# guptakhil/show-tell

Measured on AMD Instinct MI355X. Metric: training images/sec (ResNet101+GRU, emb=512, bs=128) at 1/2/4/8 MI355X, higher is better.
Workload: dtype bf16; 1 GPU; BASELINE configs[1]: ResNet-101 (train-mode BN, frozen) + 5-layer GRU decoder, E=H=512, V=10000, fwd+bwd+SGD step, synthetic COCO-shaped batch; batch_per_gpu=128, global_batch=128, image=3x224x224, parallelism=dp1

## Files before the change

include/showtell_hip.h:

```cpp
#ifndef SHOWTELL_HIP_H
#define SHOWTELL_HIP_H

#include <stddef.h>
#include <stdint.h>

#ifdef __cplusplus
extern "C" {
#endif

#define ST_F32 0
#define ST_BF16 1

#define ST_CELL_GRU 0
#define ST_CELL_LSTM 1

const char* st_last_error(void);
int st_version(void);

typedef struct {
  const void* x;
  const void* w;
  void* y;
  const float* bias;
  const float* scale;
// ... 168 lines not shown

int st_cast2d(const void* x, void* y, int from_dtype, int to_dtype, int rows, int cols, int ldx, int ldy, void* stream);

#define ST_MAX_LAYERS 8
typedef struct {
  int cell, dtype, L, in0, H, V, E;
  const void* emb;
  const void* w_ih[ST_MAX_LAYERS]; const void* w_hh[ST_MAX_LAYERS];
  const float* b_ih[ST_MAX_LAYERS]; const float* b_hh[ST_MAX_LAYERS];
  const void* w_lin; const float* b_lin;
} st_rnn_params;

typedef struct {
  float* emb;
  float* w_ih[ST_MAX_LAYERS]; float* w_hh[ST_MAX_LAYERS]; float* b_ih[ST_MAX_LAYERS]; float* b_hh[ST_MAX_LAYERS];
  float* w_lin; float* b_lin;
} st_rnn_grads;

typedef struct {
  int B, T, ntok, Tcap;
  const int* batch_sizes_host;
  const int* rows_b; const int* rows_t; const int* prev_row;
  const long* caption;
} st_packed_seq;

int st_rnn_vocab_ld(int V);
size_t st_rnn_workspace_bytes(const st_rnn_params* p, const st_packed_seq* s);
int st_rnn_forward(const st_rnn_params* p, const st_packed_seq* s, const void* x0_override, const void* feat,
                   void* workspace, size_t workspace_bytes, void* logits, int logits_dtype, int ldl,
                   long* targets, int save_for_backward, void* stream);
int st_rnn_backward(const st_rnn_params* p, const st_rnn_grads* g, const st_packed_seq* s,
                    const void* x0_override, const void* dlogits, int ldd, const float* dy_top,
                    void* workspace, size_t workspace_bytes, float* dfeat, float* dx0_out, void* stream);

int st_rnn_fused_loss_supported(const st_rnn_params* p);
size_t st_rnn_fused_loss_bytes(const st_rnn_params* p, const st_packed_seq* s);
int st_rnn_fused_loss(const st_rnn_params* p, const st_packed_seq* s, const void* workspace, size_t workspace_bytes,
                      const long* targets, float* scratch, size_t scratch_bytes, float* loss_accum, void* stream);
int st_rnn_fused_dlogits(const st_rnn_params* p, const st_packed_seq* s, const void* workspace, size_t workspace_bytes,
                         const long* targets, const float* scratch, const float* grad_scale_dev, void* dlogits, int ldd, void* stream);

int st_cross_entropy(const void* logits, int logits_dtype, const long* target, int rows, int V, int ldl,
                     float* loss_accum, void* dlogits, int dlogits_dtype, int ldd, float grad_scale,
                     const float* grad_scale_dev , void* stream);

size_t st_head_workspace_bytes(int B, int F, int E, int dtype);
int st_linear_bn1d_forward(const void* x, const void* w, const float* bias, const float* gamma, const float* beta,
                           float* running_mean, float* running_var, int B, int F, int E, int dtype,
                           int train, float momentum, float eps,
                           float* z_out, float* save_mean, float* save_rstd, void* y_dtype, float* y_f32, void* stream);
int st_linear_bn1d_backward(const float* dy, const float* z, const void* x, const float* gamma,
                            const float* save_mean, const float* save_rstd, int B, int F, int E, int dtype, int train,
                            float* dw, float* dbias, float* dgamma, float* dbeta, void* workspace, size_t workspace_bytes,
                            void* stream);

int st_sgd_step(float* param, const float* grad, float* momentum_buf, void* bf16_shadow, long n,
                float lr, float momentum, int first_step, float grad_scale, void* stream);
int st_adam_step(float* param, const float* grad, float* exp_avg, float* exp_avg_sq, void* bf16_shadow, long n,
                 float lr, float beta1, float beta2, float eps, int step, float grad_scale, void* stream);

size_t st_rnn_greedy_workspace_bytes(const st_rnn_params* p, int B);
int st_rnn_greedy(const st_rnn_params* p, const void* feat, int B, int steps, void* workspace, size_t workspace_bytes,
                  long* ids_out, float* logits_out, void* stream);
int st_rnn_greedy_last_route(void);

int st_rnn_step(const st_rnn_params* p, const void* x, int n, const void* h_in, const void* c_in,
// ... 47 lines not shown
```

show-tell_amd/_lib.py:

```python
import ctypes as C
import os

_HERE = os.path.dirname(os.path.abspath(__file__))
LIB_PATH = os.path.join(_HERE, "lib", "libshowtell_hip.so")

ST_F32, ST_BF16 = 0, 1
ST_CELL_GRU, ST_CELL_LSTM = 0, 1

c_p, c_i, c_f, c_l = C.c_void_p, C.c_int, C.c_float, C.c_long


class ConvDesc(C.Structure):
    _fields_ = [("x", c_p), ("w", c_p), ("y", c_p), ("bias", c_p), ("scale", c_p), ("shift", c_p),
                ("residual", c_p), ("stats", c_p), ("dtype", c_i), ("out_dtype", c_i),
                ("B", c_i), ("Hin", c_i), ("Win", c_i), ("Cin", c_i), ("Ho", c_i), ("Wo", c_i), ("N", c_i),
                ("KH", c_i), ("KW", c_i), ("stride", c_i), ("pad", c_i),
                ("ldx", c_i), ("ldw", c_i), ("ldy", c_i), ("relu", c_i), ("accumulate", c_i), ("Cin_logical", c_i), ("k_order", c_i), ("stats_replicas", c_i),
                ("in_stats", c_p), ("in_gamma", c_p), ("in_beta", c_p), ("in_count", c_f), ("in_eps", c_f), ("split_k", c_i)]


class Conv3x3ImgDesc(C.Structure):
    _fields_ = [("x", c_p), ("w_frag", c_p), ("y", c_p), ("stats", c_p), ("stats_replicas", c_i), ("scale", c_p), ("shift", c_p),
                ("relu", c_i), ("in_stats", c_p), ("in_gamma", c_p), ("in_beta", c_p), ("in_count", c_f), ("in_eps", c_f),
                ("B", c_i), ("H", c_i), ("W", c_i), ("C", c_i), ("N", c_i), ("in_stats_replicas", c_i)]
# ... 103 lines not shown
    "st_conv1x1_kstream": ([C.POINTER(Conv1x1WregDesc), c_p], c_i),
    "st_pack_conv_weight_frag": ([c_p, c_p, c_i, c_i, c_i, c_i, c_i, c_p], c_i),
    "st_tune": ([c_i, c_i, c_i], c_i),
    "st_prof_enable": ([c_i], c_i),
    "st_debug_stamps": ([c_p], c_i),
    "st_prof_collect": ([C.POINTER(C.c_double), C.POINTER(C.c_double), C.POINTER(c_l)], c_i),
    "st_bn_act": ([C.POINTER(BnActDesc), c_p], c_i),
    "st_bn_update_running": ([c_p, c_p, c_p, c_i, c_f, c_f, c_p], c_i),
    "st_nchw_to_nhwc": ([c_p, c_p, c_i, c_i, c_i, c_i, c_i, c_i, c_p], c_i),
    "st_nchw_to_s2d16": ([c_p, c_p, c_i, c_i, c_i, c_i, c_p], c_i),
    "st_stem_weight_s2d": ([c_p, c_p, c_i, c_i, c_p], c_i),
    "st_stem_weight_frag": ([c_p, c_p, c_p], c_i),
    "st_stem_weight_frag_packed": ([c_p, c_i, c_p, c_p], c_i),
    "st_stem_conv_pool": ([C.POINTER(StemConvPoolDesc), c_p], c_i),
    "st_nhwc_to_ncp_f32": ([c_p, c_p, c_i, c_i, c_i, c_i, c_p], c_i),
    "st_maxpool3x3s2": ([c_p, c_p, c_i, c_i, c_i, c_i, c_i, c_p], c_i),
    "st_maxpool3x3s2_bn": ([c_p, c_p, c_i, c_i, c_i, c_i, c_i, c_p, c_p, c_p, c_p, c_p, c_f, c_f, c_p], c_i),
    "st_global_avgpool": ([c_p, c_p, c_i, c_i, c_i, c_i, c_i, c_p], c_i),
    "st_cast": ([c_p, c_p, c_i, c_i, c_l, c_p], c_i),
    "st_transpose": ([c_p, c_p, c_i, c_i, c_i, c_i, c_i, c_p], c_i),
    "st_transpose_colsum": ([c_p, c_p, c_p, c_i, c_i, c_i, c_i, c_i, c_p], c_i),
    "st_transpose_batch": ([c_p, c_p, c_p, c_i, c_i, c_i, c_i, c_i, c_i, c_p, c_p, c_p], c_i),
    "st_pack_conv_weight": ([c_p, c_p, c_i, c_i, c_i, c_i, c_i, c_i, c_i, c_p], c_i),
    "st_cast2d": ([c_p, c_p, c_i, c_i, c_i, c_i, c_i, c_i, c_p], c_i),
    "st_rnn_vocab_ld": ([c_i], c_i),
    "st_rnn_workspace_bytes": ([C.POINTER(RnnParams), C.POINTER(PackedSeq)], C.c_size_t),
    "st_rnn_forward": ([C.POINTER(RnnParams), C.POINTER(PackedSeq), c_p, c_p, c_p, C.c_size_t, c_p, c_i, c_i, c_p, c_i, c_p], c_i),
    "st_rnn_fused_loss_supported": ([C.POINTER(RnnParams)], c_i),
    "st_rnn_fused_loss_bytes": ([C.POINTER(RnnParams), C.POINTER(PackedSeq)], C.c_size_t),
    "st_rnn_fused_loss": ([C.POINTER(RnnParams), C.POINTER(PackedSeq), c_p, C.c_size_t, c_p, c_p, C.c_size_t, c_p, c_p], c_i),
    "st_rnn_fused_dlogits": ([C.POINTER(RnnParams), C.POINTER(PackedSeq), c_p, C.c_size_t, c_p, c_p, c_p, c_p, c_i, c_p], c_i),
    "st_rnn_backward": ([C.POINTER(RnnParams), C.POINTER(RnnGrads), C.POINTER(PackedSeq), c_p, c_p, c_i, c_p, c_p, C.c_size_t,
                         c_p, c_p, c_p], c_i),
    "st_rnn_greedy_workspace_bytes": ([C.POINTER(RnnParams), c_i], C.c_size_t),
    "st_rnn_greedy": ([C.POINTER(RnnParams), c_p, c_i, c_i, c_p, C.c_size_t, c_p, c_p, c_p], c_i),
    "st_rnn_greedy_last_route": ([], c_i),
    "st_rnn_step": ([C.POINTER(RnnParams), c_p, c_i, c_p, c_p, c_p, c_p, c_p, c_i, c_p], c_i),
    "st_embedding_rows": ([c_p, c_p, c_p, c_i, c_i, c_i, c_i, c_i, c_p], c_i),
    "st_gather_state": ([c_p, c_p, c_p, c_i, c_i, c_i, c_i, c_i, c_p], c_i),
    "st_softmax_topk": ([c_p, c_i, c_i, c_i, c_i, c_p, c_p, c_i, c_p], c_i),
    "st_beam_select": ([c_p, c_p, c_p, c_p, c_p, c_i, c_i, c_i, c_l, c_p, c_p, c_p, c_p, c_p, c_p], c_i),
    "st_attn_workspace_bytes": ([c_p, c_p], C.c_size_t),
    "st_attn_forward": ([c_p, c_p, c_p, c_p, c_p, C.c_size_t, c_p, c_i, c_i, c_p, c_i, c_p], c_i),
    "st_attn_backward": ([c_p, c_p, c_p, c_p, c_p, c_i, c_p, c_p, c_f, c_p, c_p, C.c_size_t, c_p], c_i),
    "st_attn_reg_loss": ([c_p, c_i, c_i, c_i, c_f, c_p, c_p], c_i),
    "st_attn_greedy_workspace_bytes": ([c_p, c_i], C.c_size_t),
    "st_attn_greedy": ([c_p, c_p, c_i, c_i, c_l, c_p, C.c_size_t, c_p, c_p], c_i),
    "st_attn_greedy_alphas": ([c_p, c_p, c_i, c_i, c_l, c_p, C.c_size_t, c_p, c_p, c_p], c_i),
    "st_attn_beam_workspace_bytes": ([c_p, c_i, c_i], C.c_size_t),
    "st_attn_beam_search": ([c_p, c_p, c_i, c_i, c_i, c_l, c_l, c_p, C.c_size_t, c_p, c_p, c_p, c_p, c_p, c_p], c_i),
    "st_cross_entropy": ([c_p, c_i, c_p, c_i, c_i, c_i, c_p, c_p, c_i, c_i, c_f, c_p, c_p], c_i),
    "st_head_workspace_bytes": ([c_i, c_i, c_i, c_i], C.c_size_t),
    "st_linear_bn1d_forward": ([c_p] * 7 + [c_i, c_i, c_i, c_i, c_i, c_f, c_f] + [c_p] * 6, c_i),
    "st_linear_bn1d_backward": ([c_p] * 6 + [c_i, c_i, c_i, c_i, c_i] + [c_p] * 5 + [C.c_size_t, c_p], c_i),
    "st_sgd_step": ([c_p, c_p, c_p, c_p, c_l, c_f, c_f, c_i, c_f, c_p], c_i),
    "st_adam_step": ([c_p, c_p, c_p, c_p, c_p, c_l, c_f, c_f, c_f, c_f, c_i, c_f, c_p], c_i),
    "st_resnet_create": ([c_i, c_i, C.POINTER(c_p)], c_i),
    "st_resnet_destroy": ([c_p], None),
    "st_resnet_num_convs": ([c_p], c_i),
    "st_resnet_feat_dim": ([c_p], c_i),
    "st_resnet_weight_elems": ([c_p], C.c_size_t),
    "st_resnet_bn_channels": ([c_p], C.c_size_t),
    "st_resnet_conv_info": ([c_p, c_i] + [C.POINTER(c_i)] * 6 + [C.POINTER(C.c_size_t)] * 2 + [C.POINTER(c_i), C.POINTER(C.c_size_t), C.POINTER(c_i)], c_i),
    "st_resnet_workspace_bytes": ([c_p, c_i, c_i, c_i], C.c_size_t),
    "st_resnet_set_taps": ([c_p, c_p, C.c_size_t], c_i),
    "st_resnet_forward": ([c_p, c_p, c_i, c_i, c_i, c_p, c_p, c_p, c_p, c_p, c_i, c_f, c_f, c_p, C.c_size_t,
# ... 47 lines not shown
```

show-tell_amd/csrc/rnn.cpp:

```cpp
#include "common.h"
#include "rnn_kernels.h"
#include <string.h>
#include <vector>

namespace {

inline size_t al(size_t v) { return (v + 255) & ~(size_t)255; }
inline int up8(int v) { return (v + 7) & ~7; }

struct Plan {
  int G, GH, Np, Vp, maxw;
  size_t es;
  size_t x0, y, gates, cst, dyl, dx0, dgx, dgh, dhc, dcc, tA, tB, wT, wThh, wTih, gA, gB, total;
};

Plan make_plan(const st_rnn_params* p, const st_packed_seq* s) {
  Plan q;
  q.G = p->cell == ST_CELL_GRU ? 3 : 4;
  q.GH = q.G * p->H;
  q.Np = up8(s->ntok);
  q.Vp = st_rnn_vocab_ld(p->V);
  q.es = st_dtype_size(p->dtype);
  q.maxw = p->in0 > p->H ? p->in0 : p->H;
  const size_t n = s->ntok, L = p->L, H = p->H;
  size_t o = 0;
  auto take = [&](size_t bytes) { size_t r = o; o += al(bytes); return r; };
  q.x0 = take(n * p->in0 * q.es);
  q.y = take(L * n * H * q.es);
  q.gates = take(L * n * 4 * H * q.es);
  q.cst = take(p->cell == ST_CELL_LSTM ? L * n * H * q.es : 0);
  q.dyl = take(L * n * H * sizeof(float));
  q.dx0 = take(n * p->in0 * sizeof(float));
  q.dgx = take(L * n * q.GH * q.es);
  q.dgh = take(p->cell == ST_CELL_GRU ? L * n * q.GH * q.es : 0);
// ... 113 lines not shown
}

extern "C" int st_rnn_fused_loss_supported(const st_rnn_params* p) {
  return p && p->w_lin && p->b_lin && vocab_ce_supported(p->dtype, p->H) ? 1 : 0;
}
extern "C" size_t st_rnn_fused_loss_bytes(const st_rnn_params* p, const st_packed_seq* s) {
  if (!p || !s) return 0;
  return ((size_t)s->ntok * (2 + 2 * (size_t)vocab_ce_tiles(p->V))) * sizeof(float);
}
extern "C" int st_rnn_fused_loss(const st_rnn_params* p, const st_packed_seq* s, const void* workspace, size_t workspace_bytes,
                                 const long* targets, float* scratch, size_t scratch_bytes, float* loss_accum, void* stream) {
  if (check_common(p, s, "st_rnn_fused_loss")) return 1;
  ST_CHECK(workspace && targets && scratch && loss_accum, "st_rnn_fused_loss: null pointer");
  ST_CHECK(st_rnn_fused_loss_supported(p), "st_rnn_fused_loss: needs bf16, H = 512 and the vocabulary projection (use st_rnn_forward's logits + st_cross_entropy)");
  const Plan q = make_plan(p, s);
  ST_CHECK(workspace_bytes >= q.total && scratch_bytes >= st_rnn_fused_loss_bytes(p, s), "st_rnn_fused_loss: workspace / scratch too small");
  const char* ytop = reinterpret_cast<const char*>(workspace) + q.y + (size_t)(p->L - 1) * s->ntok * p->H * q.es;
  const int n = s->ntok;
  return vocab_ce_forward(ytop, p->w_lin, p->b_lin, targets, n, p->V, scratch + 2 * (size_t)n, scratch + n, scratch, loss_accum,
                          reinterpret_cast<hipStream_t>(stream));
}
extern "C" int st_rnn_fused_dlogits(const st_rnn_params* p, const st_packed_seq* s, const void* workspace, size_t workspace_bytes,
                                    const long* targets, const float* scratch, const float* grad_scale_dev, void* dlogits, int ldd, void* stream) {
  if (check_common(p, s, "st_rnn_fused_dlogits")) return 1;
  ST_CHECK(workspace && targets && scratch && dlogits, "st_rnn_fused_dlogits: null pointer");
  ST_CHECK(st_rnn_fused_loss_supported(p), "st_rnn_fused_dlogits: unsupported configuration");
  const Plan q = make_plan(p, s);
  ST_CHECK(workspace_bytes >= q.total, "st_rnn_fused_dlogits: workspace too small");
  const char* ytop = reinterpret_cast<const char*>(workspace) + q.y + (size_t)(p->L - 1) * s->ntok * p->H * q.es;
  return vocab_ce_dlogits(ytop, p->w_lin, p->b_lin, targets, scratch, s->ntok, p->V, dlogits, ldd, 1.0f, grad_scale_dev,
                          reinterpret_cast<hipStream_t>(stream));
}

extern "C" int st_rnn_backward(const st_rnn_params* p, const st_rnn_grads* g, const st_packed_seq* s,
                               const void* x0_override, const void* dlogits, int ldd, const float* dy_top_extra,
                               void* workspace, size_t workspace_bytes, float* dfeat, float* dx0_out, void* stream) {
  if (check_common(p, s, "st_rnn_backward")) return 1;
  ST_CHECK(g && workspace, "st_rnn_backward: null pointer");
  const Plan q = make_plan(p, s);
  ST_CHECK(workspace_bytes >= q.total, "st_rnn_backward: workspace too small (%zu < %zu)", workspace_bytes, q.total);
  hipStream_t st = reinterpret_cast<hipStream_t>(stream);
  char* ws = reinterpret_cast<char*>(workspace);
  const int dt = p->dtype, H = p->H, n = s->ntok, Np = q.Np, GH = q.GH;
  const size_t es = q.es;
  std::vector<int> off(s->T + 1, 0);
  for (int t = 0; t < s->T; ++t) off[t + 1] = off[t] + s->batch_sizes_host[t];
  const int L = p->L, T = s->T;
  auto dyl = [&](int l) { return reinterpret_cast<float*>(ws + q.dyl) + (size_t)l * n * H; };
  float* dy = dyl(L - 1);
  const char* ytop = ws + q.y + (size_t)(p->L - 1) * n * H * es;

  if (dlogits) {
    ST_CHECK(p->w_lin && g->w_lin && g->b_lin, "st_rnn_backward: vocabulary projection gradients requested without buffers");
    ST_CHECK(ldd >= up8(p->V) && ldd % 8 == 0 && ldd <= q.Vp, "st_rnn_backward: dlogits leading dimension %d must be a multiple of 8 in [%d, %d]",
             ldd, up8(p->V), q.Vp);
    if (st_transpose_colsum(dlogits, ws + q.tA, g->b_lin, dt, n, p->V, ldd, Np, stream)) return 1;
    if (st_transpose(ytop, ws + q.tB, dt, n, H, H, Np, stream)) return 1;
    if (gemm_nt(ws + q.tA, Np, ws + q.tB, Np, g->w_lin, H, p->V, H, Np, dt, ST_F32, nullptr, 1, stream)) return 1;
    if (st_transpose(p->w_lin, ws + q.wT, dt, p->V, H, H, ldd, stream)) return 1;
    const int bk = dt == ST_BF16 ? 64 : 32;
    const int split = (ldd % (8 * bk) == 0 && ldd >= 16 * bk) ? 8 : 0;
    if (gemm_nt(dlogits, ldd, ws + q.wT, ldd, dy, H, n, H, ldd, dt, ST_F32, nullptr, 0, stream, split)) return 1;
    if (dy_top_extra) { st_set_error("st_rnn_backward: dlogits and dy_top_extra are exclusive"); return 1; }
  } else {
    ST_CHECK(dy_top_extra, "st_rnn_backward: need dlogits or dy_top");
    if (hipMemcpyAsync(dy, dy_top_extra, (size_t)n * H * sizeof(float), hipMemcpyDeviceToDevice, st) != hipSuccess) {
      st_set_error("st_rnn_backward: copy failed"); return 1;
    }
  }

  const void* x0 = x0_override ? x0_override : ws + q.x0;
  const bool need_dx0 = dfeat || dx0_out || g->emb;
  float* dx0 = dx0_out ? dx0_out : reinterpret_cast<float*>(ws + q.dx0);
  const bool gru = p->cell == ST_CELL_GRU;
  auto dgxl = [&](int l) { return ws + q.dgx + (size_t)l * n * GH * es; };
  auto dghl = [&](int l) { return gru ? ws + q.dgh + (size_t)l * n * GH * es : dgxl(l); };
  auto dhcl = [&](int l) { return reinterpret_cast<float*>(ws + q.dhc) + (size_t)l * s->B * H; };
  auto dccl = [&](int l) { return reinterpret_cast<float*>(ws + q.dcc) + (size_t)l * s->B * H; };
  auto wThh = [&](int l) { return ws + q.wThh + (size_t)l * H * GH * es; };
  auto wTih = [&](int l) { return ws + q.wTih + (size_t)l * q.maxw * GH * es; };
  if (hipMemsetAsync(ws + q.dhc, 0, (size_t)L * s->B * H * sizeof(float), st) != hipSuccess ||
      hipMemsetAsync(ws + q.dcc, 0, (size_t)L * s->B * H * sizeof(float), st) != hipSuccess) { st_set_error("memset failed"); return 1; }
  {
    const void* wx[2][ST_MAX_LAYERS]; void* wy[2][ST_MAX_LAYERS];
    int ni = 0;
    for (int l = 0; l < L; ++l) {
      const int in = l == 0 ? p->in0 : H;
      wx[0][l] = p->w_hh[l]; wy[0][l] = wThh(l);
      if (!(l > 0 || need_dx0)) continue;
      if (in == H) { wx[1][ni] = p->w_ih[l]; wy[1][ni] = wTih(l); ++ni; }
      else if (st_transpose(p->w_ih[l], wTih(l), dt, GH, in, in, GH, stream)) return 1;
    }
    if (st_transpose_batch(wx[0], wy[0], nullptr, L, dt, GH, H, H, GH, nullptr, nullptr, stream)) return 1;
    if (ni && st_transpose_batch(wx[1], wy[1], nullptr, ni, dt, GH, H, H, GH, nullptr, nullptr, stream)) return 1;
  }
  for (int d = T + L - 2; d >= 0; --d) {
    RnnBwdCell gc[ST_MAX_LAYERS];
    RnnGemmArgs mc[2 * ST_MAX_LAYERS];
    int ng = 0, nm = 0;
    for (int l = d < T ? 0 : d - (T - 1); l <= d && l < L; ++l) {
      const int t = d - l;
      const int bt = s->batch_sizes_host[t];
      const int in = l == 0 ? p->in0 : H;
      char* yl = ws + q.y + (size_t)l * n * H * es;
      char* gl = ws + q.gates + (size_t)l * n * 4 * H * es;
      char* cl = ws + q.cst + (size_t)l * n * H * es;
      RnnBwdCell& c = gc[ng++];
      memset(&c, 0, sizeof(c));
      c.dy = dyl(l) + (size_t)off[t] * H; c.dhc = dhcl(l); c.dcc = dccl(l);
      c.cache = gl + (size_t)off[t] * 4 * H * es;
      c.hprev = t > 0 ? yl + (size_t)off[t - 1] * H * es : nullptr;
      c.cnew = cl + (size_t)off[t] * H * es;
      c.cprev = t > 0 ? cl + (size_t)off[t - 1] * H * es : nullptr;
      c.dgx = dgxl(l) + (size_t)off[t] * GH * es; c.dgh = dghl(l) + (size_t)off[t] * GH * es; c.Bt = bt;
      if (t > 0) {
        RnnGemmArgs& a = mc[nm++];
        memset(&a, 0, sizeof(a));
        a.A = dghl(l) + (size_t)off[t] * GH * es; a.W = wThh(l); a.M = bt; a.N = H; a.K = GH; a.lda = GH; a.ldw = GH;
        a.out_f32 = dhcl(l); a.ldo = H; a.accumulate = 1;
      }
      if (l > 0 || need_dx0) {
        RnnGemmArgs& a = mc[nm++];
        memset(&a, 0, sizeof(a));
        a.A = dgxl(l) + (size_t)off[t] * GH * es; a.W = wTih(l); a.M = bt; a.N = in; a.K = GH; a.lda = GH; a.ldw = GH;
        a.out_f32 = (l > 0 ? dyl(l - 1) + (size_t)off[t] * H : dx0 + (size_t)off[t] * in); a.ldo = in;
      }
    }
    if (rnn_bwd_gates_launch_batch(gc, ng, H, p->cell, dt, st)) return 1;
    if (rnn_gemm_launch_batch(mc, nm, dt, 0, 0, st)) return 1;
// ... 50 lines not shown
```

show-tell_amd/csrc/rnn_kernels.h:

```cpp
#pragma once
#include "common.h"

struct RnnGemmArgs {
  const void* A; const void* W; int M, N, K, lda, ldw, gstride;
  const void* A2; const void* W2; int K2, lda2, ldw2;
  float* out_f32; int ldo; int accumulate;
  const float* bias_h; const float* bias_x;
  const void* gx; int ldgx;
  const void* hprev; const void* cprev; int ldhp;
  void* hout; void* cout; int ldho;
  void* hout2; int ldho2;
  void* cache; int ldcache;
  unsigned long long* argmax_keys;
  const unsigned long long* x_keys; int x_V;
  long* ids_out; int ids_stride, ids_t;
};
constexpr int kCellRawOut = 1, kCellSplit = 2;

constexpr int kRnnBatch = 16;
struct RnnGemmBatch { RnnGemmArgs c[kRnnBatch]; };
static_assert(sizeof(RnnGemmBatch) <= 4000, "kernel-argument segment is 4 KiB");
struct RnnBwdCell {
  const float* dy; float* dhc; float* dcc; const void* cache; const void* hprev; const void* cnew; const void* cprev;
  void* dgx; void* dgh; int Bt;
};
struct RnnBwdBatch { RnnBwdCell c[kRnnBatch]; };

#ifdef __HIPCC__
__device__ __forceinline__ float st_sigm(float x) { return 1.0f / (1.0f + expf(-x)); }
__device__ __forceinline__ float st_gru_unit(float xr, float xz, float xn, float hr, float hz, float hn, float hprev, float& r, float& z, float& n) {
  r = st_sigm(xr + hr);
  z = st_sigm(xz + hz);
  n = tanhf(__builtin_fmaf(r, hn, xn));
  return __builtin_fmaf(z, hprev, (1.f - z) * n);
}
__device__ __forceinline__ float st_lstm_unit(float pi, float pf, float pg, float po, float cprev, float& ig, float& fg, float& gg, float& og, float& cn) {
  ig = st_sigm(pi); fg = st_sigm(pf); gg = tanhf(pg); og = st_sigm(po);
  cn = __builtin_fmaf(fg, cprev, ig * gg);
  return og * tanhf(cn);
}
#endif

size_t rnn_greedy_pipe_bytes(const st_rnn_params* p, int B, int steps);
int rnn_greedy_pipe(const st_rnn_params* p, const void* feat, int B, int steps, void* ws, size_t ws_bytes, long* ids_out, hipStream_t st);

int vocab_ce_supported(int dtype, int H);
int vocab_ce_tiles(int V);
int vocab_ce_forward(const void* y, const void* w, const float* bias, const long* target, int n, int V, float* partial, float* tgt,
                     float* lse, float* loss, hipStream_t st);
int vocab_ce_dlogits(const void* y, const void* w, const float* bias, const long* target, const float* lse, int n, int V,
                     void* dlogits, int ldd, float gscale, const float* gscale_dev, hipStream_t st);

int rnn_gemm_launch(const RnnGemmArgs& a, int dtype, int epi, int has_x, hipStream_t st);
int rnn_gemm_launch_batch(const RnnGemmArgs* cells, int ncells, int dtype, int epi, int has_x, hipStream_t st);
int rnn_bwd_gates_launch_batch(const RnnBwdCell* cells, int ncells, int H, int cell_kind, int dtype, hipStream_t st);
int pack_inputs_launch(const void* feat, const void* emb, const long* cap, int Tcap, const int* rows_b, const int* rows_t,
                       void* x0, long* target, int ntok, int E, int V, int mode, int dtype, hipStream_t st);
int embedding_bwd_launch(const float* dx0, const long* cap, int Tcap, const int* rows_b, const int* rows_t,
                         float* dfeat, float* demb, int ntok, int E, int V, int mode, hipStream_t st);
int gather_hprev_launch(const void* y, const int* rows_t, const int* prev_row, void* hp, int ntok, int H, int dtype, hipStream_t st,
                        const void* h0 = nullptr, const int* rows_b = nullptr);
int gru_bwd_gates_launch(const float* dy, float* dhc, const void* cache, const void* hprev, void* dgx, void* dgh,
                         int Bt, int H, int dtype, hipStream_t st);
int lstm_bwd_gates_launch(const float* dy, float* dhc, float* dcc, const void* cache, const void* cnew, const void* cprev,
                          void* dg, int Bt, int H, int dtype, hipStream_t st);
int colsum_launch(const void* x, float* out, int rows, int cols, int ldx, int dtype, hipStream_t st);
```

show-tell_amd/csrc/rnn_kernels.hip:

```cpp
#include "common.h"
#include "rnn_kernels.h"
#include <string.h>

namespace {

template <typename T> struct Mfma;
template <> struct Mfma<bf16_t> {
  static constexpr int EPC = 8;
  static __device__ __forceinline__ void run(const u32x4& a, const u32x4& b, f32x4& c) {
    c = __builtin_amdgcn_mfma_f32_16x16x32_bf16(*reinterpret_cast<const bf16x8*>(&a),
                                                *reinterpret_cast<const bf16x8*>(&b), c, 0, 0, 0);
  }
};
template <> struct Mfma<float> {
  static constexpr int EPC = 4;
  static __device__ __forceinline__ void run(const u32x4& a, const u32x4& b, f32x4& c) {
#pragma unroll
    for (int e = 0; e < 4; ++e)
      c = __builtin_amdgcn_mfma_f32_16x16x4f32(__uint_as_float(a[e]), __uint_as_float(b[e]), c, 0, 0, 0);
  }
};

template <typename T> __device__ __forceinline__ void load4(const T* p, float* v);
template <> __device__ __forceinline__ void load4<float>(const float* p, float* v) {
  const f32x4 t = *reinterpret_cast<const f32x4*>(p);
  v[0] = t[0]; v[1] = t[1]; v[2] = t[2]; v[3] = t[3];
}
template <> __device__ __forceinline__ void load4<bf16_t>(const bf16_t* p, float* v) {
  const u32x2 t = *reinterpret_cast<const u32x2*>(p);
  v[0] = __uint_as_float(t[0] << 16); v[1] = __uint_as_float(t[0] & 0xffff0000u);
  v[2] = __uint_as_float(t[1] << 16); v[3] = __uint_as_float(t[1] & 0xffff0000u);
}
template <typename T> __device__ __forceinline__ void store4(T* p, const float* v);
template <> __device__ __forceinline__ void store4<float>(float* p, const float* v) {
  *reinterpret_cast<f32x4*>(p) = f32x4{v[0], v[1], v[2], v[3]};
}
template <> __device__ __forceinline__ void store4<bf16_t>(bf16_t* p, const float* v) {
  *reinterpret_cast<u32x2*>(p) = u32x2{pack_bf16x2(v[0], v[1]), pack_bf16x2(v[2], v[3])};
}

__device__ __forceinline__ float sigm(float x) { return 1.0f / (1.0f + expf(-x)); }

template <typename T, int NG, bool HAS_X, int MT>
__device__ __forceinline__ void skinny_mma(const RnnGemmArgs& a, int mbase, int n0, int r16, int q4, int kslice,
                                           f32x4 (&accH)[MT][NG], f32x4 (&accX)[MT][NG]) {
  constexpr int EPC = Mfma<T>::EPC;
  constexpr int UNR = (HAS_X && MT == 2) ? 2 : 4;
  const int n = n0 + r16;
  const bool nok = n < a.N;
  const bool hasH = a.A != nullptr, hasX = HAS_X && a.A2 != nullptr;
  const T* WH = reinterpret_cast<const T*>(a.W) + (long)n * a.ldw;
  const long gsH = (long)a.gstride * a.ldw;
  const T* WX = reinterpret_cast<const T*>(a.W2) + (long)n * a.ldw2;
  const long gsX = (long)a.gstride * a.ldw2;
  const T* AH[MT]; const T* AX[MT]; bool mok[MT];
#pragma unroll
  for (int t = 0; t < MT; ++t) {
    const int m = mbase + t * 16 + r16;
    mok[t] = m < a.M;
    AH[t] = reinterpret_cast<const T*>(a.A) + (long)m * a.lda;
    if (!HAS_X && a.x_keys && a.A) {
      int tok = 0;
      if (mok[t]) {
        tok = (int)(0xffffffffu - (unsigned)(a.x_keys[m] & 0xffffffffull));
        if (tok < 0 || tok >= a.x_V) tok = 0;
        if (a.ids_out && n0 == 0 && kslice == 0 && q4 == 0) a.ids_out[(long)m * a.ids_stride + a.ids_t] = tok;
      }
      AH[t] = reinterpret_cast<const T*>(a.A) + (long)tok * a.lda;
    }
    long xrow = m;
    if (HAS_X && a.x_keys) {
      int tok = 0;
      if (mok[t]) {
        tok = (int)(0xffffffffu - (unsigned)(a.x_keys[m] & 0xffffffffull));
        if (tok < 0 || tok >= a.x_V) tok = 0;
        if (a.ids_out && n0 == 0 && kslice == 0 && q4 == 0) a.ids_out[(long)m * a.ids_stride + a.ids_t] = tok;
      }
      xrow = tok;
    }
    AX[t] = reinterpret_cast<const T*>(a.A2) + xrow * a.lda2;
  }
  const int nsH = hasH ? (a.K + 4 * EPC - 1) / (4 * EPC) : 0, nsX = hasX ? (a.K2 + 4 * EPC - 1) / (4 * EPC) : 0;
  const int spwH = (nsH + 3) / 4, spwX = (nsX + 3) / 4;
  const int begH = kslice * spwH, endH = min(nsH, begH + spwH), begX = kslice * spwX, endX = min(nsX, begX + spwX);
  const int ngroups = max((endH - begH + UNR - 1) / UNR, (endX - begX + UNR - 1) / UNR);
  for (int gi = 0; gi < ngroups; ++gi) {
    u32x4 fa[MT][UNR], fw[UNR][NG], xa[MT][UNR], xw[UNR][NG];
#pragma unroll
    for (int u = 0; u < UNR; ++u) {
      const int sH = begH + gi * UNR + u, kH = (sH * 4 + q4) * EPC;
      const bool okH = sH < endH && kH < a.K;
#pragma unroll
      for (int t = 0; t < MT; ++t) {
        fa[t][u] = u32x4{0u, 0u, 0u, 0u};
        if (mok[t] && okH) fa[t][u] = *reinterpret_cast<const u32x4*>(AH[t] + kH);
      }
#pragma unroll
      for (int g = 0; g < NG; ++g) {
        fw[u][g] = u32x4{0u, 0u, 0u, 0u};
        if (nok && okH) fw[u][g] = *reinterpret_cast<const u32x4*>(WH + g * gsH + kH);
      }
      if (HAS_X) {
        const int sX = begX + gi * UNR + u, kX = (sX * 4 + q4) * EPC;
        const bool okX = sX < endX && kX < a.K2;
#pragma unroll
        for (int t = 0; t < MT; ++t) {
          xa[t][u] = u32x4{0u, 0u, 0u, 0u};
          if (mok[t] && okX) xa[t][u] = *reinterpret_cast<const u32x4*>(AX[t] + kX);
        }
#pragma unroll
        for (int g = 0; g < NG; ++g) {
          xw[u][g] = u32x4{0u, 0u, 0u, 0u};
          if (nok && okX) xw[u][g] = *reinterpret_cast<const u32x4*>(WX + g * gsX + kX);
        }
      }
    }
#pragma unroll
    for (int u = 0; u < UNR; ++u)
#pragma unroll
      for (int g = 0; g < NG; ++g)
#pragma unroll
        for (int t = 0; t < MT; ++t) {
          Mfma<T>::run(fw[u][g], fa[t][u], accH[t][g]);
          if (HAS_X) Mfma<T>::run(xw[u][g], xa[t][u], accX[t][g]);
        }
  }
}

template <typename T, int NG, int EPI, bool HAS_X, int MT>
__global__ __launch_bounds__(256) void rnn_gemm_kernel(RnnGemmBatch batch) {
  const RnnGemmArgs& a = batch.c[blockIdx.z];
  __shared__ f32x4 red[4][MT][2 * NG][64];
  const int lane = threadIdx.x & 63;
  const int wid = __builtin_amdgcn_readfirstlane(threadIdx.x >> 6);
  const int r16 = lane & 15, q4 = lane >> 4;
  const int n0 = blockIdx.x * 16, mbase = blockIdx.y * 16 * MT;
  if (mbase >= a.M || n0 >= a.N) return;
  const int m0 = mbase + (wid < MT ? wid : 0) * 16;
  f32x4 accH[MT][NG], accX[MT][NG];
#pragma unroll
  for (int t = 0; t < MT; ++t)
#pragma unroll
    for (int g = 0; g < NG; ++g) { accH[t][g] = f32x4{0.f, 0.f, 0.f, 0.f}; accX[t][g] = f32x4{0.f, 0.f, 0.f, 0.f}; }
  const int pm = m0 + r16, pn = n0 + 4 * q4;
  const bool epi_ok = wid < MT && pm < a.M && pn < a.N && EPI != 3;
  float ex[NG][4], eb[NG][4], es[4] = {0.f, 0.f, 0.f, 0.f};
#pragma unroll
  for (int g = 0; g < NG; ++g)
#pragma unroll
    for (int e = 0; e < 4; ++e) { ex[g][e] = 0.f; eb[g][e] = 0.f; }
  if (epi_ok) {
    if (EPI == 0) {
      if (a.bias_h) load4<float>(a.bias_h + pn, eb[0]);
      if (a.accumulate) load4<float>(a.out_f32 + (long)pm * a.ldo + pn, es);
    } else {
#pragma unroll
      for (int g = 0; g < NG; ++g) {
        load4<float>(a.bias_h + g * a.N + pn, eb[g]);
        if (HAS_X) load4<float>(a.bias_x + g * a.N + pn, ex[g]);
        else if (a.accumulate == kCellSplit) load4<float>(reinterpret_cast<const float*>(a.gx) + (long)pm * a.ldgx + g * a.N + pn, ex[g]);
        else if (a.accumulate != kCellRawOut) load4<T>(reinterpret_cast<const T*>(a.gx) + (long)pm * a.ldgx + g * a.N + pn, ex[g]);
      }
      const void* prev = EPI == 1 ? a.hprev : a.cprev;
      if (prev && a.accumulate != kCellRawOut) load4<T>(reinterpret_cast<const T*>(prev) + (long)pm * a.ldhp + pn, es);
    }
  }
  skinny_mma<T, NG, HAS_X, MT>(a, mbase, n0, r16, q4, wid, accH, accX);
#pragma unroll
  for (int t = 0; t < MT; ++t)
#pragma unroll
    for (int g = 0; g < NG; ++g) { red[wid][t][g][lane] = accH[t][g]; if (HAS_X) red[wid][t][NG + g][lane] = accX[t][g]; }
  __syncthreads();
  if (wid >= MT) return;
  f32x4 sumH[NG], sumX[NG];
#pragma unroll
  for (int g = 0; g < NG; ++g) {
    sumH[g] = red[0][wid][g][lane];
    if (HAS_X) sumX[g] = red[0][wid][NG + g][lane];
#pragma unroll
    for (int w = 1; w < 4; ++w) {
      sumH[g] += red[w][wid][g][lane];
      if (HAS_X) sumX[g] += red[w][wid][NG + g][lane];
    }
  }

  const int m = m0 + r16, n = n0 + 4 * q4;
  if (EPI != 3 && (m >= a.M || n >= a.N)) return;
  const int H = a.N;
  if (EPI == 3) {
    float best = -INFINITY; int bi = 0x7fffffff;
#pragma unroll
    for (int e = 0; e < 4; ++e) {
      if (n + e < a.N) {
        const float v = sumH[0][e] + (a.bias_h ? a.bias_h[n + e] : 0.f);
        if (v > best) { best = v; bi = n + e; }
      }
    }
#pragma unroll
    for (int o = 16; o < 64; o <<= 1) {
      const float ov = __shfl_xor(best, o, 64); const int oi = __shfl_xor(bi, o, 64);
// ... 107 lines not shown
                                                           const T* __restrict__ h0, const int* __restrict__ rows_b) {
  constexpr int N = 16 / (int)sizeof(T);
  const int cpr = H / N;
  const long total = (long)ntok * cpr;
  for (long i = (long)blockIdx.x * blockDim.x + threadIdx.x; i < total; i += (long)gridDim.x * blockDim.x) {
    const int row = (int)(i / cpr), c = (int)(i - (long)row * cpr) * N;
    u32x4 v = {0u, 0u, 0u, 0u};
    if (rows_t[row] > 0) v = *reinterpret_cast<const u32x4*>(y + (long)prev_row[row] * H + c);
    else if (h0) v = *reinterpret_cast<const u32x4*>(h0 + (long)rows_b[row] * H + c);
    *reinterpret_cast<u32x4*>(hp + (long)row * H + c) = v;
  }
}

template <typename T>
__global__ __launch_bounds__(256) void gru_bwd_gates_kernel(RnnBwdBatch batch, int H) {
  const RnnBwdCell& cl = batch.c[blockIdx.y];
  const float* __restrict__ dy = cl.dy; float* __restrict__ dhc = cl.dhc;
  const T* __restrict__ cache = reinterpret_cast<const T*>(cl.cache);
  const T* __restrict__ hprev = reinterpret_cast<const T*>(cl.hprev);
  T* __restrict__ dgx = reinterpret_cast<T*>(cl.dgx); T* __restrict__ dgh = reinterpret_cast<T*>(cl.dgh);
  const int Bt = cl.Bt;
  const int total = Bt * (H / 4);
  const int i = blockIdx.x * blockDim.x + threadIdx.x;
  if (i >= total) return;
  const int b = i / (H / 4), j = (i - b * (H / 4)) * 4;
  float g[4], c[4], r[4], z[4], n[4], hn[4], hp[4] = {0.f, 0.f, 0.f, 0.f};
  load4<float>(dy + (long)b * H + j, g);
  load4<float>(dhc + (long)b * H + j, c);
  const T* cr = cache + (long)b * 4 * H + j;
  load4<T>(cr, r); load4<T>(cr + H, z); load4<T>(cr + 2 * H, n); load4<T>(cr + 3 * H, hn);
  if (hprev) load4<T>(hprev + (long)b * H + j, hp);
  float drp[4], dzp[4], dnp[4], dnr[4], dhz[4];
#pragma unroll
  for (int e = 0; e < 4; ++e) {
    const float dh = g[e] + c[e];
    const float dn = dh * (1.f - z[e]);
    const float dz = dh * (hp[e] - n[e]);
    dnp[e] = dn * (1.f - n[e] * n[e]);
    drp[e] = dnp[e] * hn[e] * r[e] * (1.f - r[e]);
    dzp[e] = dz * z[e] * (1.f - z[e]);
    dnr[e] = dnp[e] * r[e];
    dhz[e] = dh * z[e];
  }
  T* ox = dgx + (long)b * 3 * H + j;
  T* oh = dgh + (long)b * 3 * H + j;
  store4<T>(ox, drp); store4<T>(ox + H, dzp); store4<T>(ox + 2 * H, dnp);
  store4<T>(oh, drp); store4<T>(oh + H, dzp); store4<T>(oh + 2 * H, dnr);
  store4<float>(dhc + (long)b * H + j, dhz);
}

template <typename T>
__global__ __launch_bounds__(256) void lstm_bwd_gates_kernel(RnnBwdBatch batch, int H) {
  const RnnBwdCell& cl = batch.c[blockIdx.y];
  const float* __restrict__ dy = cl.dy; float* __restrict__ dhc = cl.dhc; float* __restrict__ dcc = cl.dcc;
  const T* __restrict__ cache = reinterpret_cast<const T*>(cl.cache);
  const T* __restrict__ cnew = reinterpret_cast<const T*>(cl.cnew);
  const T* __restrict__ cprev = reinterpret_cast<const T*>(cl.cprev);
  T* __restrict__ dg = reinterpret_cast<T*>(cl.dgx);
  const int Bt = cl.Bt;
  const int total = Bt * (H / 4);
  const int i = blockIdx.x * blockDim.x + threadIdx.x;
  if (i >= total) return;
  const int b = i / (H / 4), j = (i - b * (H / 4)) * 4;
  float g[4], ch[4], cc[4], ig[4], fg[4], gg[4], og[4], cn[4], cp[4] = {0.f, 0.f, 0.f, 0.f};
  load4<float>(dy + (long)b * H + j, g);
  load4<float>(dhc + (long)b * H + j, ch);
  load4<float>(dcc + (long)b * H + j, cc);
  const T* cr = cache + (long)b * 4 * H + j;
  load4<T>(cr, ig); load4<T>(cr + H, fg); load4<T>(cr + 2 * H, gg); load4<T>(cr + 3 * H, og);
  load4<T>(cnew + (long)b * H + j, cn);
  if (cprev) load4<T>(cprev + (long)b * H + j, cp);
  float di[4], df[4], dgg[4], dob[4], dcp[4], zero[4] = {0.f, 0.f, 0.f, 0.f};
#pragma unroll
  for (int e = 0; e < 4; ++e) {
    const float dh = g[e] + ch[e];
    const float tc = tanhf(cn[e]);
    const float dc = cc[e] + dh * og[e] * (1.f - tc * tc);
    dob[e] = dh * tc * og[e] * (1.f - og[e]);
    di[e] = dc * gg[e] * ig[e] * (1.f - ig[e]);
    df[e] = dc * cp[e] * fg[e] * (1.f - fg[e]);
    dgg[e] = dc * ig[e] * (1.f - gg[e] * gg[e]);
// ... 99 lines not shown
  }
#undef RG
  ST_LAUNCH_CHECK();
  return 0;
}

int rnn_gemm_launch(const RnnGemmArgs& a, int dtype, int epi, int has_x, hipStream_t st) {
  return rnn_gemm_launch_batch(&a, 1, dtype, epi, has_x, st);
}

int rnn_bwd_gates_launch_batch(const RnnBwdCell* cells, int ncells, int H, int cell_kind, int dtype, hipStream_t st) {
  ST_CHECK(ncells >= 0 && ncells <= kRnnBatch, "rnn_bwd_gates: %d cells in one launch (max %d)", ncells, kRnnBatch);
  RnnBwdBatch b;
  memset(&b, 0, sizeof(b));
  int nc = 0, maxB = 0;
  for (int i = 0; i < ncells; ++i) {
    if (cells[i].Bt <= 0) continue;
    b.c[nc++] = cells[i];
    if (cells[i].Bt > maxB) maxB = cells[i].Bt;
  }
  if (nc == 0) return 0;
  const dim3 grid((maxB * (H / 4) + 255) / 256, nc);
  if (cell_kind == ST_CELL_GRU) {
    if (dtype == ST_BF16) hipLaunchKernelGGL(gru_bwd_gates_kernel<bf16_t>, grid, dim3(256), 0, st, b, H);
    else hipLaunchKernelGGL(gru_bwd_gates_kernel<float>, grid, dim3(256), 0, st, b, H);
  } else {
    if (dtype == ST_BF16) hipLaunchKernelGGL(lstm_bwd_gates_kernel<bf16_t>, grid, dim3(256), 0, st, b, H);
    else hipLaunchKernelGGL(lstm_bwd_gates_kernel<float>, grid, dim3(256), 0, st, b, H);
  }
  ST_LAUNCH_CHECK();
  return 0;
}

static inline int grid1d(long work, int threads = 256) {
  long b = (work + threads - 1) / threads;
  return (int)(b < 1 ? 1 : (b > 4096 ? 4096 : b));
}

int pack_inputs_launch(const void* feat, const void* emb, const long* cap, int Tcap, const int* rows_b, const int* rows_t,
                       void* x0, long* target, int ntok, int E, int V, int mode, int dtype, hipStream_t st) {
  if (ntok <= 0) return 0;
  const int n = dtype == ST_BF16 ? 8 : 4;
  ST_CHECK(E % n == 0, "pack_inputs: E=%d must be a multiple of %d", E, n);
  const int grid = grid1d((long)ntok * (E / n));
  if (dtype == ST_BF16) hipLaunchKernelGGL(pack_inputs_kernel<bf16_t>, dim3(grid), dim3(256), 0, st, (const bf16_t*)feat, (const bf16_t*)emb, cap, Tcap, rows_b, rows_t, (bf16_t*)x0, target, ntok, E, V, mode);
  else hipLaunchKernelGGL(pack_inputs_kernel<float>, dim3(grid), dim3(256), 0, st, (const float*)feat, (const float*)emb, cap, Tcap, rows_b, rows_t, (float*)x0, target, ntok, E, V, mode);
  ST_LAUNCH_CHECK();
  return 0;
}

int embedding_bwd_launch(const float* dx0, const long* cap, int Tcap, const int* rows_b, const int* rows_t,
                         float* dfeat, float* demb, int ntok, int E, int V, int mode, hipStream_t st) {
  if (ntok <= 0) return 0;
  hipLaunchKernelGGL(embedding_bwd_kernel, dim3(grid1d((long)ntok * E)), dim3(256), 0, st, dx0, cap, Tcap, rows_b, rows_t, dfeat, demb, ntok, E, V, mode);
  ST_LAUNCH_CHECK();
  return 0;
}

int gather_hprev_launch(const void* y, const int* rows_t, const int* prev_row, void* hp, int ntok, int H, int dtype, hipStream_t st,
                        const void* h0, const int* rows_b) {
  if (ntok <= 0) return 0;
  const int n = dtype == ST_BF16 ? 8 : 4;
  ST_CHECK(H % n == 0, "gather_hprev: H=%d must be a multiple of %d", H, n);
  const int grid = grid1d((long)ntok * (H / n));
  if (dtype == ST_BF16) hipLaunchKernelGGL(gather_hprev_kernel<bf16_t>, dim3(grid), dim3(256), 0, st, (const bf16_t*)y, rows_t, prev_row, (bf16_t*)hp, ntok, H, (const bf16_t*)h0, rows_b);
  else hipLaunchKernelGGL(gather_hprev_kernel<float>, dim3(grid), dim3(256), 0, st, (const float*)y, rows_t, prev_row, (float*)hp, ntok, H, (const float*)h0, rows_b);
// ... 51 lines not shown
```

Measured before the change: 31830 images/sec.

## Fuse GRU backward-through-time GEMMs and gate gradients into one per-wavefront kernel

Adds a fused GRU BPTT kernel that, per diagonal wavefront of (layer, time) cells, computes the recurrent dh GEMM (dgh_next·WhhT) and the upward dx GEMM (dgx_up·WihT) with MFMA, reduces across waves in shared memory, and applies the GRU gate backward in the epilogue. It is on by default for GRU and can be turned off with ST_BPTT_FUSED=0. It also drops the carry memsets and issues a single large GEMM for dx0 at the end. The aim is fewer launches and fewer round trips of intermediate gradients through global memory on the sequential critical path. The cost is that each block does a K=3H reduction with little parallelism, which may use fewer CUs than the separate batched GEMMs.

```diff
diff --git a/include/showtell_hip.h b/include/showtell_hip.h
--- a/include/showtell_hip.h
+++ b/include/showtell_hip.h
@@ -224,6 +224,7 @@
 int st_rnn_backward(const st_rnn_params* p, const st_rnn_grads* g, const st_packed_seq* s,
                     const void* x0_override, const void* dlogits, int ldd, const float* dy_top,
                     void* workspace, size_t workspace_bytes, float* dfeat, float* dx0_out, void* stream);
+int st_rnn_backward_last_route(void);
 
 int st_rnn_fused_loss_supported(const st_rnn_params* p);
 size_t st_rnn_fused_loss_bytes(const st_rnn_params* p, const st_packed_seq* s);
diff --git a/show-tell_amd/_lib.py b/show-tell_amd/_lib.py
--- a/show-tell_amd/_lib.py
+++ b/show-tell_amd/_lib.py
@@ -159,6 +159,7 @@
     "st_rnn_fused_dlogits": ([C.POINTER(RnnParams), C.POINTER(PackedSeq), c_p, C.c_size_t, c_p, c_p, c_p, c_p, c_i, c_p], c_i),
     "st_rnn_backward": ([C.POINTER(RnnParams), C.POINTER(RnnGrads), C.POINTER(PackedSeq), c_p, c_p, c_i, c_p, c_p, C.c_size_t,
                          c_p, c_p, c_p], c_i),
+    "st_rnn_backward_last_route": ([], c_i),
     "st_rnn_greedy_workspace_bytes": ([C.POINTER(RnnParams), c_i], C.c_size_t),
     "st_rnn_greedy": ([C.POINTER(RnnParams), c_p, c_i, c_i, c_p, C.c_size_t, c_p, c_p, c_p], c_i),
     "st_rnn_greedy_last_route": ([], c_i),
diff --git a/show-tell_amd/csrc/rnn.cpp b/show-tell_amd/csrc/rnn.cpp
--- a/show-tell_amd/csrc/rnn.cpp
+++ b/show-tell_amd/csrc/rnn.cpp
@@ -1,5 +1,6 @@
 #include "common.h"
 #include "rnn_kernels.h"
+#include <stdlib.h>
 #include <string.h>
 #include <vector>
 
@@ -179,6 +180,9 @@
                           reinterpret_cast<hipStream_t>(stream));
 }
 
+static thread_local int g_bptt_route = 0;
+extern "C" int st_rnn_backward_last_route(void) { return g_bptt_route; }
+
 extern "C" int st_rnn_backward(const st_rnn_params* p, const st_rnn_grads* g, const st_packed_seq* s,
                                const void* x0_override, const void* dlogits, int ldd, const float* dy_top_extra,
                                void* workspace, size_t workspace_bytes, float* dfeat, float* dx0_out, void* stream) {
@@ -226,8 +230,11 @@
   auto dccl = [&](int l) { return reinterpret_cast<float*>(ws + q.dcc) + (size_t)l * s->B * H; };
   auto wThh = [&](int l) { return ws + q.wThh + (size_t)l * H * GH * es; };
   auto wTih = [&](int l) { return ws + q.wTih + (size_t)l * q.maxw * GH * es; };
-  if (hipMemsetAsync(ws + q.dhc, 0, (size_t)L * s->B * H * sizeof(float), st) != hipSuccess ||
-      hipMemsetAsync(ws + q.dcc, 0, (size_t)L * s->B * H * sizeof(float), st) != hipSuccess) { st_set_error("memset failed"); return 1; }
+  const char* env = getenv("ST_BPTT_FUSED");
+  const bool fused = gru && (!env || atoi(env) != 0);
+  g_bptt_route = fused ? 1 : 0;
+  if (!fused && (hipMemsetAsync(ws + q.dhc, 0, (size_t)L * s->B * H * sizeof(float), st) != hipSuccess ||
+                 hipMemsetAsync(ws + q.dcc, 0, (size_t)L * s->B * H * sizeof(float), st) != hipSuccess)) { st_set_error("memset failed"); return 1; }
   {
     const void* wx[2][ST_MAX_LAYERS]; void* wy[2][ST_MAX_LAYERS];
     int ni = 0;
@@ -241,7 +248,34 @@
     if (st_transpose_batch(wx[0], wy[0], nullptr, L, dt, GH, H, H, GH, nullptr, nullptr, stream)) return 1;
     if (ni && st_transpose_batch(wx[1], wy[1], nullptr, ni, dt, GH, H, H, GH, nullptr, nullptr, stream)) return 1;
   }
-  for (int d = T + L - 2; d >= 0; --d) {
+  for (int d = T + L - 2; fused && d >= 0; --d) {
+    RnnBpttCell bc[ST_MAX_LAYERS];
+    int nb = 0;
+    for (int l = d < T ? 0 : d - (T - 1); l <= d && l < L; ++l) {
+      const int t = d - l;
+      RnnBpttCell& c = bc[nb++];
+      memset(&c, 0, sizeof(c));
+      c.Mx = s->batch_sizes_host[t];
+      c.Mh = t + 1 < T ? s->batch_sizes_host[t + 1] : 0;
+      if (c.Mh > 0) c.dgh_next = dghl(l) + (size_t)off[t + 1] * GH * es;
+      c.wThh = wThh(l);
+      if (l + 1 < L) { c.dgx_up = dgxl(l + 1) + (size_t)off[t] * GH * es; c.wTih = wTih(l + 1); }
+      else c.dy_top = dy + (size_t)off[t] * H;
+      c.carry = dhcl(l);
+      c.cache = ws + q.gates + ((size_t)l * n + off[t]) * 4 * H * es;
+      c.hprev = t > 0 ? ws + q.y + ((size_t)l * n + off[t - 1]) * H * es : nullptr;
+      c.dgx = dgxl(l) + (size_t)off[t] * GH * es; c.dgh = dghl(l) + (size_t)off[t] * GH * es;
+    }
+    if (gru_bptt_launch_batch(bc, nb, H, dt, st)) return 1;
+  }
+  if (fused && need_dx0) {
+    RnnGemmArgs a;
+    memset(&a, 0, sizeof(a));
+    a.A = dgxl(0); a.W = wTih(0); a.M = n; a.N = p->in0; a.K = GH; a.lda = GH; a.ldw = GH;
+    a.out_f32 = dx0; a.ldo = p->in0;
+    if (rnn_gemm_launch(a, dt, 0, 0, st)) return 1;
+  }
+  for (int d = T + L - 2; !fused && d >= 0; --d) {
     RnnBwdCell gc[ST_MAX_LAYERS];
     RnnGemmArgs mc[2 * ST_MAX_LAYERS];
     int ng = 0, nm = 0;
diff --git a/show-tell_amd/csrc/rnn_kernels.h b/show-tell_amd/csrc/rnn_kernels.h
--- a/show-tell_amd/csrc/rnn_kernels.h
+++ b/show-tell_amd/csrc/rnn_kernels.h
@@ -25,6 +25,16 @@
   void* dgx; void* dgh; int Bt;
 };
 struct RnnBwdBatch { RnnBwdCell c[kRnnBatch]; };
+struct RnnBpttCell {
+  const void* dgh_next; const void* wThh;
+  const void* dgx_up; const void* wTih;
+  const float* dy_top;
+  float* carry;
+  const void* cache; const void* hprev;
+  void* dgx; void* dgh;
+  int Mh, Mx;
+};
+struct RnnBpttBatch { RnnBpttCell c[ST_MAX_LAYERS]; int H; };
 
 #ifdef __HIPCC__
 __device__ __forceinline__ float st_sigm(float x) { return 1.0f / (1.0f + expf(-x)); }
@@ -38,6 +48,17 @@
   ig = st_sigm(pi); fg = st_sigm(pf); gg = tanhf(pg); og = st_sigm(po);
   cn = __builtin_fmaf(fg, cprev, ig * gg);
   return og * tanhf(cn);
+}
+__device__ __forceinline__ void st_gru_bwd_unit(float dy, float dhc, float r, float z, float n, float hn, float hp,
+                                                float& drp, float& dzp, float& dnp, float& dnr, float& dhz) {
+  const float dh = dy + dhc;
+  const float dn = dh * (1.f - z);
+  const float dz = dh * (hp - n);
+  dnp = dn * __builtin_fmaf(-n, n, 1.f);
+  drp = dnp * hn * r * (1.f - r);
+  dzp = dz * z * (1.f - z);
+  dnr = dnp * r;
+  dhz = dh * z;
 }
 #endif
 
@@ -54,6 +75,7 @@
 int rnn_gemm_launch(const RnnGemmArgs& a, int dtype, int epi, int has_x, hipStream_t st);
 int rnn_gemm_launch_batch(const RnnGemmArgs* cells, int ncells, int dtype, int epi, int has_x, hipStream_t st);
 int rnn_bwd_gates_launch_batch(const RnnBwdCell* cells, int ncells, int H, int cell_kind, int dtype, hipStream_t st);
+int gru_bptt_launch_batch(const RnnBpttCell* cells, int ncells, int H, int dtype, hipStream_t st);
 int pack_inputs_launch(const void* feat, const void* emb, const long* cap, int Tcap, const int* rows_b, const int* rows_t,
                        void* x0, long* target, int ntok, int E, int V, int mode, int dtype, hipStream_t st);
 int embedding_bwd_launch(const float* dx0, const long* cap, int Tcap, const int* rows_b, const int* rows_t,
diff --git a/show-tell_amd/csrc/rnn_kernels.hip b/show-tell_amd/csrc/rnn_kernels.hip
--- a/show-tell_amd/csrc/rnn_kernels.hip
+++ b/show-tell_amd/csrc/rnn_kernels.hip
@@ -43,7 +43,7 @@
 
 template <typename T, int NG, bool HAS_X, int MT>
 __device__ __forceinline__ void skinny_mma(const RnnGemmArgs& a, int mbase, int n0, int r16, int q4, int kslice,
-                                           f32x4 (&accH)[MT][NG], f32x4 (&accX)[MT][NG]) {
+                                           f32x4 (&accH)[MT][NG], f32x4 (&accX)[MT][NG], int MX) {
   constexpr int EPC = Mfma<T>::EPC;
   constexpr int UNR = (HAS_X && MT == 2) ? 2 : 4;
   const int n = n0 + r16;
@@ -53,11 +53,12 @@
   const long gsH = (long)a.gstride * a.ldw;
   const T* WX = reinterpret_cast<const T*>(a.W2) + (long)n * a.ldw2;
   const long gsX = (long)a.gstride * a.ldw2;
-  const T* AH[MT]; const T* AX[MT]; bool mok[MT];
+  const T* AH[MT]; const T* AX[MT]; bool mok[MT], mokX[MT];
 #pragma unroll
   for (int t = 0; t < MT; ++t) {
     const int m = mbase + t * 16 + r16;
     mok[t] = m < a.M;
+    mokX[t] = m < MX;
     AH[t] = reinterpret_cast<const T*>(a.A) + (long)m * a.lda;
     if (!HAS_X && a.x_keys && a.A) {
       int tok = 0;
@@ -106,7 +107,7 @@
 #pragma unroll
         for (int t = 0; t < MT; ++t) {
           xa[t][u] = u32x4{0u, 0u, 0u, 0u};
-          if (mok[t] && okX) xa[t][u] = *reinterpret_cast<const u32x4*>(AX[t] + kX);
+          if (mokX[t] && okX) xa[t][u] = *reinterpret_cast<const u32x4*>(AX[t] + kX);
         }
 #pragma unroll
         for (int g = 0; g < NG; ++g) {
@@ -165,7 +166,7 @@
       if (prev && a.accumulate != kCellRawOut) load4<T>(reinterpret_cast<const T*>(prev) + (long)pm * a.ldhp + pn, es);
     }
   }
-  skinny_mma<T, NG, HAS_X, MT>(a, mbase, n0, r16, q4, wid, accH, accX);
+  skinny_mma<T, NG, HAS_X, MT>(a, mbase, n0, r16, q4, wid, accH, accX, a.M);
 #pragma unroll
   for (int t = 0; t < MT; ++t)
 #pragma unroll
@@ -339,21 +340,63 @@
   if (hprev) load4<T>(hprev + (long)b * H + j, hp);
   float drp[4], dzp[4], dnp[4], dnr[4], dhz[4];
 #pragma unroll
-  for (int e = 0; e < 4; ++e) {
-    const float dh = g[e] + c[e];
-    const float dn = dh * (1.f - z[e]);
-    const float dz = dh * (hp[e] - n[e]);
-    dnp[e] = dn * (1.f - n[e] * n[e]);
-    drp[e] = dnp[e] * hn[e] * r[e] * (1.f - r[e]);
-    dzp[e] = dz * z[e] * (1.f - z[e]);
-    dnr[e] = dnp[e] * r[e];
-    dhz[e] = dh * z[e];
-  }
+  for (int e = 0; e < 4; ++e) st_gru_bwd_unit(g[e], c[e], r[e], z[e], n[e], hn[e], hp[e], drp[e], dzp[e], dnp[e], dnr[e], dhz[e]);
   T* ox = dgx + (long)b * 3 * H + j;
   T* oh = dgh + (long)b * 3 * H + j;
   store4<T>(ox, drp); store4<T>(ox + H, dzp); store4<T>(ox + 2 * H, dnp);
   store4<T>(oh, drp); store4<T>(oh + H, dzp); store4<T>(oh + 2 * H, dnr);
   store4<float>(dhc + (long)b * H + j, dhz);
+}
+
+template <typename T, int MT>
+__global__ __launch_bounds__(256) void gru_bptt_cell_kernel(RnnBpttBatch batch) {
+  const RnnBpttCell& c = batch.c[blockIdx.z];
+  const int H = batch.H;
+  __shared__ f32x4 red[4][MT][2][64];
+  const int lane = threadIdx.x & 63;
+  const int wid = __builtin_amdgcn_readfirstlane(threadIdx.x >> 6);
+  const int r16 = lane & 15, q4 = lane >> 4;
+  const int n0 = blockIdx.x * 16, mbase = blockIdx.y * 16 * MT;
+  if (mbase >= c.Mx || n0 >= H) return;
+  const int m0 = mbase + (wid < MT ? wid : 0) * 16;
+  const int m = m0 + r16, n = n0 + 4 * q4;
+  const bool epi_ok = wid < MT && m < c.Mx && n < H;
+  const bool has_carry = m < c.Mh;
+  float dy[4] = {0.f, 0.f, 0.f, 0.f}, cr[4] = {0.f, 0.f, 0.f, 0.f}, hp[4] = {0.f, 0.f, 0.f, 0.f}, r[4], z[4], nn[4], hn[4];
+  if (epi_ok) {
+    if (!c.dgx_up) load4<float>(c.dy_top + (long)m * H + n, dy);
+    if (has_carry) load4<float>(c.carry + (long)m * H + n, cr);
+    const T* g = reinterpret_cast<const T*>(c.cache) + (long)m * 4 * H + n;
+    load4<T>(g, r); load4<T>(g + H, z); load4<T>(g + 2 * H, nn); load4<T>(g + 3 * H, hn);
+    if (c.hprev) load4<T>(reinterpret_cast<const T*>(c.hprev) + (long)m * H + n, hp);
+  }
+  RnnGemmArgs a;
+  a.A = c.Mh > 0 ? c.dgh_next : nullptr; a.W = c.wThh; a.M = c.Mh; a.N = H; a.K = 3 * H; a.lda = 3 * H; a.ldw = 3 * H; a.gstride = 0;
+  a.A2 = c.dgx_up; a.W2 = c.wTih; a.K2 = 3 * H; a.lda2 = 3 * H; a.ldw2 = 3 * H;
+  a.x_keys = nullptr; a.x_V = 0; a.ids_out = nullptr; a.ids_stride = 0; a.ids_t = 0;
+  f32x4 accH[MT][1], accX[MT][1];
+#pragma unroll
+  for (int t = 0; t < MT; ++t) { accH[t][0] = f32x4{0.f, 0.f, 0.f, 0.f}; accX[t][0] = f32x4{0.f, 0.f, 0.f, 0.f}; }
+  skinny_mma<T, 1, true, MT>(a, mbase, n0, r16, q4, wid, accH, accX, c.Mx);
+#pragma unroll
+  for (int t = 0; t < MT; ++t) { red[wid][t][0][lane] = accH[t][0]; red[wid][t][1][lane] = accX[t][0]; }
+  __syncthreads();
+  if (!epi_ok) return;
+  f32x4 sumH = red[0][wid][0][lane], sumX = red[0][wid][1][lane];
+#pragma unroll
+  for (int w = 1; w < 4; ++w) { sumH += red[w][wid][0][lane]; sumX += red[w][wid][1][lane]; }
+  float drp[4], dzp[4], dnp[4], dnr[4], dhz[4];
+#pragma unroll
+  for (int e = 0; e < 4; ++e) {
+    const float dyl = c.dgx_up ? (sumX[e] + 0.f) + 0.f : dy[e];
+    const float dhc = has_carry ? (sumH[e] + 0.f) + cr[e] : 0.f;
+    st_gru_bwd_unit(dyl, dhc, r[e], z[e], nn[e], hn[e], hp[e], drp[e], dzp[e], dnp[e], dnr[e], dhz[e]);
+  }
+  T* ox = reinterpret_cast<T*>(c.dgx) + (long)m * 3 * H + n;
+  T* oh = reinterpret_cast<T*>(c.dgh) + (long)m * 3 * H + n;
+  store4<T>(ox, drp); store4<T>(ox + H, dzp); store4<T>(ox + 2 * H, dnp);
+  store4<T>(oh, drp); store4<T>(oh + H, dzp); store4<T>(oh + 2 * H, dnr);
+  store4<float>(c.carry + (long)m * H + n, dhz);
 }
 
 template <typename T>
@@ -519,6 +562,36 @@
   return 0;
 }
 
+int gru_bptt_launch_batch(const RnnBpttCell* cells, int ncells, int H, int dtype, hipStream_t st) {
+  ST_CHECK(ncells >= 0 && ncells <= ST_MAX_LAYERS, "gru_bptt: %d cells in one launch (max %d)", ncells, ST_MAX_LAYERS);
+  const int epc = dtype == ST_BF16 ? 8 : 4;
+  ST_CHECK(H % epc == 0, "gru_bptt: H=%d must be a multiple of %d", H, epc);
+  RnnBpttBatch b;
+  memset(&b, 0, sizeof(b));
+  b.H = H;
+  int nc = 0, maxM = 0;
+  for (int i = 0; i < ncells; ++i) {
+    const RnnBpttCell& c = cells[i];
+    if (c.Mx <= 0) continue;
+    ST_CHECK(c.Mh >= 0 && c.Mh <= c.Mx && (c.Mh == 0 || c.dgh_next) && (c.dgx_up || c.dy_top) && c.wThh && (!c.dgx_up || c.wTih) &&
+             c.carry && c.cache && c.dgx && c.dgh, "gru_bptt: bad cell descriptor");
+    b.c[nc++] = c;
+    if (c.Mx > maxM) maxM = c.Mx;
+  }
+  if (nc == 0) return 0;
+  const bool mt2 = (nc >= 2 || maxM >= 512) && maxM > 16;
+  const dim3 grid((H + 15) / 16, (maxM + 15) / 16, nc), grid2((H + 15) / 16, (maxM + 31) / 32, nc), block(256);
+  if (dtype == ST_BF16) {
+    if (mt2) hipLaunchKernelGGL((gru_bptt_cell_kernel<bf16_t, 2>), grid2, block, 0, st, b);
+    else hipLaunchKernelGGL((gru_bptt_cell_kernel<bf16_t, 1>), grid, block, 0, st, b);
+  } else {
+    if (mt2) hipLaunchKernelGGL((gru_bptt_cell_kernel<float, 2>), grid2, block, 0, st, b);
+    else hipLaunchKernelGGL((gru_bptt_cell_kernel<float, 1>), grid, block, 0, st, b);
+  }
+  ST_LAUNCH_CHECK();
+  return 0;
+}
+
 static inline int grid1d(long work, int threads = 256) {
   long b = (work + threads - 1) / threads;
   return (int)(b < 1 ? 1 : (b > 4096 ? 4096 : b));
```

Result: no change. 31650 images/sec (-0.6%).
